# Rintazero/ft8_demodulator

Hardware: AMD Instinct MI355X
Metric: 15-s FT8 slots/sec (full decode) + LDPC candidates/sec, 1/2/4/8 MI355X (higher is better)
Workload: dtype f32 (STFT, sync score) / f64 (LLR, BP); 1 GPU; BASELINE config 3: batch of 256 independent 15-s slots per GPU, 12 kHz, K=300 candidates, min_score=2, 20 BP iterations (config 5 shape at N>1); slots_per_gpu=256, max_candidates=300, min_score=2, pipeline_depth=2, parallelism=slot-sharded x1

## Files before the change

### ft8_demodulator_amd/csrc/bp.hip

```cpp
#include "ft8_internal.h"
#include "heap_replay.h"

namespace ft8 {
namespace {

__constant__ uint16_t kChkStartD[FT8_LDPC_M + 1] = FT8_CHK_START_INIT;
__constant__ uint8_t kEdgeVarD[FT8_LDPC_E] = FT8_EDGE_VAR_INIT;
__constant__ uint16_t kVarEdgeD[FT8_LDPC_N * 3] = FT8_VAR_EDGE_INIT;
__constant__ uint8_t kEdgeChkD[FT8_LDPC_E] = FT8_EDGE_CHK_INIT;
constexpr int kGrayD[8] = {0, 1, 3, 2, 5, 6, 4, 7};

constexpr int kEdgeSlots = (FT8_LDPC_E + kWave - 1) / kWave;
constexpr int kVarSlots = (FT8_LDPC_N + kWave - 1) / kWave;
constexpr int kChkSlots = (FT8_LDPC_M + kWave - 1) / kWave;

constexpr int kDivGroup = 3;
static_assert(kEdgeSlots % kDivGroup == 0 && kVarSlots == kDivGroup, "division groups tile the slots exactly");
constexpr int kProdGroup = 3;
static_assert(kEdgeSlots % kProdGroup == 0, "product groups tile the edge slots");
constexpr int kBpWavesPerSimd = 4;
constexpr int kBpLbWaves = 3;
constexpr int kBpGridCus = 256;
constexpr double kClip2 = 2.0 * 4.97;

typedef __attribute__((address_space(3))) const double lds_f64;
typedef __attribute__((address_space(3))) const uint64_t lds_u64;

__device__ double sqrt_rn(double x) {
  double y = __builtin_sqrt(x);
  if (!(x > 0.0) || __builtin_isinf(x)) return y;
  for (int it = 0; it < 4; ++it) {
    const double lo = __longlong_as_double(__double_as_longlong(y) - 1);
    const double hi = __longlong_as_double(__double_as_longlong(y) + 1);
    if (__builtin_fma(y, lo, -x) >= 0.0) { y = lo; continue; }
    if (__builtin_fma(y, hi, -x) < 0.0) { y = hi; continue; }
    break;
  }
  return y;
}

__device__ __forceinline__ double pymax4(double a, double b, double c, double d) {
  double m = a;
  m = b > m ? b : m;
  m = c > m ? c : m;
  m = d > m ? d : m;
  return m;
}

template <int N>
__device__ __forceinline__ void div_fast(double* q, const double* x, const double* y) {
  double r[N], e[N], m[N];
#pragma unroll
  for (int i = 0; i < N; ++i) r[i] = __builtin_amdgcn_rcp(y[i]);
#pragma unroll
  for (int i = 0; i < N; ++i) e[i] = __builtin_fma(-y[i], r[i], 1.0);
#pragma unroll
  for (int i = 0; i < N; ++i) r[i] = __builtin_fma(r[i], e[i], r[i]);
#pragma unroll
  for (int i = 0; i < N; ++i) e[i] = __builtin_fma(-y[i], r[i], 1.0);
#pragma unroll
  for (int i = 0; i < N; ++i) r[i] = __builtin_fma(r[i], e[i], r[i]);
#pragma unroll
  for (int i = 0; i < N; ++i) m[i] = x[i] * r[i];
#pragma unroll
  for (int i = 0; i < N; ++i) e[i] = __builtin_fma(-y[i], m[i], x[i]);
#pragma unroll
  for (int i = 0; i < N; ++i) q[i] = __builtin_fma(e[i], r[i], m[i]);
}

template <int N, bool NEG2 = false>
__device__ __forceinline__ void div_rn(double* q, const double* x, const double* y_in, int fast = 0) {
  int ok = fast;
  if (!ok) {
    double mn = __builtin_fabs(x[0]);
#pragma unroll
    for (int i = 1; i < N; ++i) mn = __builtin_fmin(mn, __builtin_fabs(x[i]));
    ok = __ballot(mn >= 0x1p-960) == __builtin_amdgcn_read_exec() ? 1 : 0;
  }
  double r[N], e[N], m[N];
  if (ok) {
#pragma unroll
    for (int i = 0; i < N; ++i) r[i] = __builtin_amdgcn_rcp(y_in[i]);
#pragma unroll
    for (int i = 0; i < N; ++i) e[i] = __builtin_fma(-y_in[i], r[i], 1.0);
#pragma unroll
    for (int i = 0; i < N; ++i) r[i] = __builtin_fma(r[i], e[i], r[i]);
#pragma unroll
    for (int i = 0; i < N; ++i) e[i] = __builtin_fma(-y_in[i], r[i], 1.0);
#pragma unroll
    for (int i = 0; i < N; ++i) r[i] = __builtin_fma(r[i], e[i], r[i]);
#pragma unroll
    for (int i = 0; i < N; ++i) m[i] = x[i] * r[i];
#pragma unroll
    for (int i = 0; i < N; ++i) e[i] = __builtin_fma(-y_in[i], m[i], x[i]);
#pragma unroll
    for (int i = 0; i < N; ++i) q[i] = __builtin_fma(e[i], r[i], m[i]);
    return;
  }
  double den[N], num[N], y[N];
  bool f0[N], f1[N];
#pragma unroll
  for (int i = 0; i < N; ++i) y[i] = NEG2 ? -2.0 * y_in[i] : y_in[i];
#pragma unroll
  for (int i = 0; i < N; ++i) den[i] = __builtin_amdgcn_div_scale(x[i], y[i], false, &f0[i]);
#pragma unroll
  for (int i = 0; i < N; ++i) r[i] = __builtin_amdgcn_rcp(den[i]);
#pragma unroll
  for (int i = 0; i < N; ++i) num[i] = __builtin_amdgcn_div_scale(x[i], y[i], true, &f1[i]);
#pragma unroll
  for (int i = 0; i < N; ++i) e[i] = __builtin_fma(-den[i], r[i], 1.0);
#pragma unroll
  for (int i = 0; i < N; ++i) r[i] = __builtin_fma(r[i], e[i], r[i]);
#pragma unroll
  for (int i = 0; i < N; ++i) e[i] = __builtin_fma(-den[i], r[i], 1.0);
#pragma unroll
  for (int i = 0; i < N; ++i) r[i] = __builtin_fma(r[i], e[i], r[i]);
#pragma unroll
  for (int i = 0; i < N; ++i) m[i] = num[i] * r[i];
#pragma unroll
  for (int i = 0; i < N; ++i) e[i] = __builtin_fma(-den[i], m[i], num[i]);
#pragma unroll
  for (int i = 0; i < N; ++i) q[i] = __builtin_amdgcn_div_fmas(e[i], r[i], m[i], f1[i]);
#pragma unroll
  for (int i = 0; i < N; ++i) q[i] = __builtin_amdgcn_div_fixup(q[i], y[i], x[i]);
  if constexpr (NEG2) {
#pragma unroll
    for (int i = 0; i < N; ++i) q[i] = -2.0 * q[i];
  }
  (void)f0;
}

constexpr int kM7 = 24;
constexpr int kQS = FT8_LDPC_M;
constexpr int kQ6 = 6 * kQS;
constexpr int kMsgN = 584;
constexpr int kOne = kMsgN - 1;
constexpr int kHdr = 1024;
static_assert(kEdgeSlots * kWave <= kMsgN && kQ6 + kM7 == FT8_LDPC_E, "row-major message layout");

__host__ __device__ constexpr int q_of(int idx) { return idx < kQ6 ? idx / kQS : 6; }
__host__ __device__ constexpr int qa_of(int i) { return q_of(kWave * i); }
__host__ __device__ constexpr bool mixed_slot(int i) { return q_of(kWave * i + kWave - 1) != q_of(kWave * i); }
__host__ __device__ constexpr int hi_lane(int i) { return kQS * (qa_of(i) + 1) - kWave * i; }
__host__ __device__ constexpr int row_off(int i) { return 8 * (kWave * i - kQS * qa_of(i)); }

struct WaveLds {
  uint8_t bits[256];
  uint8_t a91[16];
  uint8_t rank[FT8_LDPC_M];
  uint8_t chk_of[FT8_LDPC_M];
  uint8_t pad_[kHdr - 256 - 16 - 2 * FT8_LDPC_M];
  double msg[kMsgN];
};
static_assert(offsetof(WaveLds, msg) == kHdr, "msg follows the header");

struct WaveTables {
  uint32_t va[kVarSlots], va1[kVarSlots];
  uint32_t vb[kVarSlots];
  uint32_t h[kChkSlots][kVarSlots][2];
};

__device__ __forceinline__ double ldv(uint32_t addr) {
  return *(const volatile __attribute__((address_space(3))) double*)(uintptr_t)addr;
}

__device__ __forceinline__ uint32_t lds_addr(const void* p) {
  return (uint32_t)(uintptr_t)(__attribute__((address_space(3))) const void*)p;
}

__device__ void load_tables(WaveTables& t, WaveLds& L, int lane) {
  if (lane == 0) {
    int c7 = 0, c6 = kM7;
    for (int m = 0; m < FT8_LDPC_M; ++m) {
      const int r = (kChkStartD[m + 1] - kChkStartD[m]) == 7 ? c7++ : c6++;
      L.rank[m] = (uint8_t)r;
      L.chk_of[r] = (uint8_t)m;
    }
  }
  __syncthreads();
  const uint32_t msg0 = lds_addr(&L.msg[0]);
  auto addr_of = [&](int e) -> uint32_t {
    const int m = kEdgeChkD[e], q = e - kChkStartD[m], r = L.rank[m];
    return msg0 + 8u * (uint32_t)(q < 6 ? q * kQS + r : kQ6 + r);
  };
#pragma unroll
  for (int j = 0; j < kVarSlots; ++j) {
    const int n = lane + kWave * j;
    if (n < FT8_LDPC_N) {
      t.va[j] = addr_of(kVarEdgeD[3 * n]);
      t.va1[j] = addr_of(kVarEdgeD[3 * n + 1]);
      t.vb[j] = addr_of(kVarEdgeD[3 * n + 2]);
    } else {
      const uint32_t one = msg0 + 8u * kOne;
      t.va[j] = t.va1[j] = one;
      t.vb[j] = one;
    }
  }
#pragma unroll
  for (int k = 0; k < kChkSlots; ++k) {
    const int mp = lane + kWave * k;
#pragma unroll
    for (int j = 0; j < kVarSlots; ++j) t.h[k][j][0] = t.h[k][j][1] = 0;
    if (mp < FT8_LDPC_M) {
      const int m = L.chk_of[mp];
      for (int e = kChkStartD[m]; e < kChkStartD[m + 1]; ++e) {
        const int v = kEdgeVarD[e];
#pragma unroll
        for (int j = 0; j < kVarSlots; ++j)
#pragma unroll
          for (int w = 0; w < 2; ++w)
            if (v >> 5 == 2 * j + w) t.h[k][j][w] |= 1u << (v & 31);
      }
    }
  }
  for (int x = FT8_LDPC_E + lane; x < kMsgN; x += kWave) L.msg[x] = 1.0;
  __syncthreads();
#pragma unroll
  for (int j = 0; j < kVarSlots; ++j) asm volatile("" : "+v"(t.va[j]), "+v"(t.vb[j]));
#pragma unroll
  for (int j = 0; j < kVarSlots; ++j) asm volatile("" : "+v"(t.va1[j]));
#pragma unroll
  for (int k = 0; k < kChkSlots; ++k)
#pragma unroll
    for (int j = 0; j < kVarSlots; ++j) asm volatile("" : "+v"(t.h[k][j][0]), "+v"(t.h[k][j][1]));
}

struct BpArgs {
  const void* wf;
  int wf_f64, T, F, sps, bpt, num_blocks;
  const int32_t* cand;
  const double* cand_score;
  const int32_t* cand_count;
  int N, n_items, mode, n_slots;
  const double* llr_in;
  int normalize, max_iterations;
  double* llr_out;
  uint8_t* plain_out;
  ft8_result* res;
  unsigned long long* work;
  unsigned long long work_base;
  unsigned long long* stats;
  unsigned long long* clock;
  int slot0;
  int tie_blocks;
  TieArgs tie;
};

__device__ bool tie_order(const TieArgs& a, int slot) {
  if (slot >= a.n_slots) return false;
  const int w = a.warn[slot];
  if (!(w & 8)) return false;
  const int lane = threadIdx.x, N = a.N;
  const int nsel = __builtin_amdgcn_readfirstlane(a.cand_count[slot]);
  int32_t* t = a.tie + (int64_t)slot * tie_stride(N);
  const int32_t* push = t;
  const int32_t* sel = t + N;
  int32_t* perm = t + 2 * N;
  int32_t* mi = t + 3 * N;
  int32_t* mp = t + 4 * N;
  int32_t* mk = t + 5 * N;
  const int rec = t[7 * N];
  const float* psc = reinterpret_cast<const float*>(t + 7 * N + 2);
  const double* ssc = a.cand_score + (int64_t)slot * N;
  unsigned hh[kReplayRegs], hl[kReplayRegs];
  heap_load(psc, push, nsel, hh, hl);
  int tie = heap_pushes(nsel, hh, hl);
  if (rec >= 0) tie |= heap_record(nsel, hh, hl, mono_neg(__int_as_float(t[7 * N + 1])), (unsigned)rec);

  int M = 0;
  for (int i0 = 0; i0 < nsel; i0 += kWave) {
    const int i = i0 + lane;
    unsigned key = 0, idx = 0;
    bool mem = false;
    if (i < nsel) {
      idx = (unsigned)sel[i];
      key = mono_neg((float)ssc[i]);
      mem = (i > 0 && mono_neg((float)ssc[i - 1]) == key) || (i + 1 < nsel && mono_neg((float)ssc[i + 1]) == key);
    }
    unsigned long long b = __ballot(mem);
    while (b) {
      const int l = __ffsll((long long)b) - 1;
      b &= b - 1;
      const unsigned sl = rdl(idx, l), kl = rdl(key, l);
      unsigned P = 0;
#pragma unroll
      for (int k = 0; k < kReplayRegs; ++k) {
        const int pos = 64 * k + lane;
        const unsigned long long m = __ballot(pos >= 1 && pos <= nsel && hl[k] == sl);
        if (m) P = 64u * k + (unsigned)(__ffsll((long long)m) - 1);
      }
      if (lane == 0) {
        mi[M] = i0 + l;
        mp[M] = (int)P;
        mk[M] = (int)kl;
      }
      ++M;
    }
  }
  for (int i = lane; i < nsel; i += kWave) perm[i] = i;
  __syncthreads();
  for (int m = lane; m < M; m += kWave) {
    const int i = mi[m], P = mp[m], K = mk[m];
    int below_i = 0, below_p = 0;
    for (int j = 0; j < M; ++j) {
      if (mk[j] == K) {
        below_i += mi[j] < i;
        below_p += mp[j] < P;
      }
    }
    perm[i - below_i + below_p] = i;
  }
  if (lane == 0 && tie) a.warn[slot] = w | 1;
  return true;
}

__global__ __launch_bounds__(kWave) void k_tie_apply(TieArgs a, int32_t* cand, double* cand_score) {
  const int slot = blockIdx.x, lane = threadIdx.x, N = a.N;
  if (!tie_order(a, slot)) return;
  __syncthreads();
  const int nsel = a.cand_count[slot];
  int32_t* t = a.tie + (int64_t)slot * tie_stride(N);
  const int32_t* perm = t + 2 * N;
  int32_t* stage = t + 3 * N;
  int32_t* cs = cand + (int64_t)slot * N * 2;
  double* ss = cand_score + (int64_t)slot * N;
  for (int i = lane; i < nsel; i += kWave) {
    const int src = perm[i];
    stage[4 * i] = cs[2 * src];
    stage[4 * i + 1] = cs[2 * src + 1];
    const long long v = __double_as_longlong(ss[src]);
    stage[4 * i + 2] = (int32_t)v;
    stage[4 * i + 3] = (int32_t)(v >> 32);
  }
  __syncthreads();
  for (int i = lane; i < nsel; i += kWave) {
    cs[2 * i] = stage[4 * i];
    cs[2 * i + 1] = stage[4 * i + 1];
    ss[i] = __longlong_as_double(((long long)stage[4 * i + 3] << 32) | (unsigned)stage[4 * i + 2]);
  }
}

constexpr int kLlrCpw = 4;
constexpr int kLlrRow = FT8_LDPC_N + 2;

__device__ double pairwise174x4(const double (*x)[kLlrRow], double (*part)[16], int lane) {
  const int u = lane >> 4, l = lane & 15;
  const double* xu = x[u];
  double r;
  if (l < 8) {
    r = xu[l];
    for (int i = 8; i < 80; i += 8) r += xu[i + l];
  } else {
    const int j = l - 8;
    r = xu[80 + j];
    for (int i = 8; i < 88; i += 8) r += xu[80 + i + j];
  }
  part[u][l] = r;
  __syncthreads();
  double tot = 0.0;
  if (l == 0) {
    const double* pu = part[u];
    const double s1 = ((pu[0] + pu[1]) + (pu[2] + pu[3])) + ((pu[4] + pu[5]) + (pu[6] + pu[7]));
    double s2 = ((pu[8] + pu[9]) + (pu[10] + pu[11])) + ((pu[12] + pu[13]) + (pu[14] + pu[15]));
    for (int i = 168; i < 174; ++i) s2 += xu[i];
    tot = 0.0 + (s1 + s2);
  }
  __syncthreads();
  return __shfl(tot, lane & ~15);
}

template <typename T>
__device__ void extract_llr_x4(const BpArgs& a, const int (&slot)[kLlrCpw], const int (&at)[kLlrCpw],
                               const int (&af)[kLlrCpw], int n_on, double (*c)[kLlrRow], T (*stage)[64 * 8],
                               int lane) {
  const int i = lane & 7, g = lane >> 3;
  const T* wf0 = reinterpret_cast<const T*>(a.wf);
  T v[kLlrCpw][8];
#pragma unroll
  for (int u = 0; u < kLlrCpw; ++u) {
    const int base = floordiv(at[u], a.sps);
    const T* wf = wf0 + (int64_t)slot[u] * a.T * a.F;
#pragma unroll
    for (int r = 0; r < 8; ++r) {
      const int k = 8 * r + g;
      const int sym = k + (k < 29 ? 7 : 14);
      const int block = base + sym;
      v[u][r] = (T)0;
      if (u < n_on && k < 58 && !(block < 0 || block >= a.num_blocks))
        v[u][r] = wf[(int64_t)(at[u] + sym * a.sps) * a.F + af[u] + i * a.bpt];
    }
  }
#pragma unroll
  for (int u = 0; u < kLlrCpw; ++u)
#pragma unroll
    for (int r = 0; r < 8; ++r) stage[u][8 * (8 * r + g) + i] = v[u][r];
  __syncthreads();
  if (lane < 58) {
    const int k = lane;
    const int sym = k + (k < 29 ? 7 : 14);
#pragma unroll
    for (int u = 0; u < kLlrCpw; ++u) {
      if (u >= n_on) break;
      const int block = floordiv(at[u], a.sps) + sym;
      double l0 = 0.0, l1 = 0.0, l2 = 0.0;
      if (!(block < 0 || block >= a.num_blocks)) {
        double s[8], s2[8];
#pragma unroll
        for (int j = 0; j < 8; ++j) s[j] = (double)stage[u][8 * k + j];
#pragma unroll
        for (int j = 0; j < 8; ++j) s2[j] = s[kGrayD[j]];
        l0 = pymax4(s2[4], s2[5], s2[6], s2[7]) - pymax4(s2[0], s2[1], s2[2], s2[3]);
        l1 = pymax4(s2[2], s2[3], s2[6], s2[7]) - pymax4(s2[0], s2[1], s2[4], s2[5]);
        l2 = pymax4(s2[1], s2[3], s2[5], s2[7]) - pymax4(s2[0], s2[2], s2[4], s2[6]);
      }
      c[u][3 * k] = l0;
      c[u][3 * k + 1] = l1;
      c[u][3 * k + 2] = l2;
    }
  }
}

template <typename T>
__global__ __launch_bounds__(kWave) void k_llr(BpArgs a) {
  __shared__ double c[kLlrCpw][kLlrRow];
  __shared__ double part[kLlrCpw][16];
  __shared__ double bc[kLlrCpw];
  constexpr size_t kScratch = sizeof(T) * kLlrCpw * 64 * 8 > sizeof(double) * kLlrCpw * kLlrRow
                                  ? sizeof(T) * kLlrCpw * 64 * 8 : sizeof(double) * kLlrCpw * kLlrRow;
  __shared__ __attribute__((aligned(16))) unsigned char scratch[kScratch];
  double (*sq)[kLlrRow] = reinterpret_cast<double (*)[kLlrRow]>(scratch);
  const int lane = threadIdx.x;
  if ((int)blockIdx.x < a.tie_blocks) {
    tie_order(a.tie, blockIdx.x);
    return;
  }
  const int id = blockIdx.x - a.tie_blocks;
  int item0, n_on;
  int slot[kLlrCpw] = {0, 0, 0, 0}, at[kLlrCpw] = {0, 0, 0, 0}, af[kLlrCpw] = {0, 0, 0, 0};
  static_assert(kLlrCpw == 4, "four candidates per wave");
  if (a.mode == 0) {
    const int groups = (a.N + kLlrCpw - 1) / kLlrCpw;
    const int q = id >> 3;
    const int s0 = (q / groups) * 8 + (id & 7);
    const int c0 = (q % groups) * kLlrCpw;
    if (s0 >= a.n_slots) return;
    n_on = min(kLlrCpw, min(a.N, a.cand_count[s0]) - c0);
    item0 = s0 * a.N + c0;
#pragma unroll
    for (int u = 0; u < kLlrCpw; ++u) {
      slot[u] = s0;
      if (u < n_on) {
        at[u] = a.cand[((int64_t)item0 + u) * 2];
        af[u] = a.cand[((int64_t)item0 + u) * 2 + 1];
      }
    }
  } else {
    item0 = id * kLlrCpw;
    n_on = min(kLlrCpw, a.n_items - item0);
    if (a.mode == 1) {
#pragma unroll
      for (int u = 0; u < kLlrCpw; ++u) {
        if (u < n_on) {
          slot[u] = a.cand[((int64_t)item0 + u) * 3];
          at[u] = a.cand[((int64_t)item0 + u) * 3 + 1];
          af[u] = a.cand[((int64_t)item0 + u) * 3 + 2];
        }
      }
    }
  }
  if (n_on <= 0) return;
  if (a.mode == 2) {
    for (int e = lane; e < n_on * FT8_LDPC_N; e += kWave) {
      const int u = e / FT8_LDPC_N, n = e - u * FT8_LDPC_N;
      c[u][n] = a.llr_in[(int64_t)(item0 + u) * FT8_LDPC_N + n];
    }
  } else {
    extract_llr_x4<T>(a, slot, at, af, n_on, c, reinterpret_cast<T (*)[64 * 8]>(scratch), lane);
  }
  __syncthreads();
  if (a.normalize) {
    const double mean = pairwise174x4(c, part, lane) / 174.0;
    if ((lane & 15) == 0) bc[lane >> 4] = mean;
    __syncthreads();
    for (int e = lane; e < n_on * FT8_LDPC_N; e += kWave) {
      const int u = e / FT8_LDPC_N, n = e - u * FT8_LDPC_N;
      const double d = c[u][n] - bc[u];
      sq[u][n] = d * d;
    }
    __syncthreads();
    const double var = pairwise174x4(sq, part, lane) / 174.0;
    if ((lane & 15) == 0) bc[lane >> 4] = sqrt_rn(24.0 / var);
    __syncthreads();
    for (int e = lane; e < n_on * FT8_LDPC_N; e += kWave) {
      const int u = e / FT8_LDPC_N, n = e - u * FT8_LDPC_N;
      a.llr_out[(int64_t)(item0 + u) * FT8_LDPC_N + n] = c[u][n] * bc[u];
    }
    return;
  }
  for (int e = lane; e < n_on * FT8_LDPC_N; e += kWave) {
    const int u = e / FT8_LDPC_N, n = e - u * FT8_LDPC_N;
    a.llr_out[(int64_t)(item0 + u) * FT8_LDPC_N + n] = c[u][n];
  }
}

__device__ __forceinline__ void sweep_sync() { asm volatile("" ::: "memory"); }

__device__ __forceinline__ double clip2(double T, bool nan_in) {
  const double y = __builtin_fmin(__builtin_fmax(T, -kClip2), kClip2);
  return (nan_in && T != T) ? T : y;
}

__device__ __forceinline__ void tanh_group(double* v, int fast = 0) {
  double na[kDivGroup], nb[kDivGroup];
#pragma unroll
  for (int i = 0; i < kDivGroup; ++i) {
    const double yv = v[i], z = yv * yv;
    na[i] = yv * (15120.0 + z * (420.0 + z));
    nb[i] = -30240.0 + z * (-3360.0 + z * -30.0);
  }
  int ok = fast;
  if (!ok) {
    double mn = INFINITY;
#pragma unroll
    for (int i = 0; i < kDivGroup; ++i) mn = __builtin_fmin(mn, __builtin_fabs(na[i]));
    ok = __ballot(mn >= 0x1p-480) == __builtin_amdgcn_read_exec() ? 1 : 0;
  }
  if (ok) {
    div_fast<kDivGroup>(v, na, nb);
  } else {
#pragma unroll
    for (int i = 0; i < kDivGroup; ++i) {
      const double xv = -0.5 * v[i], x2 = xv * xv;
      na[i] = xv * (945.0 + x2 * (105.0 + x2));
      nb[i] = 945.0 + x2 * (420.0 + x2 * 15.0);
    }
    div_rn<kDivGroup>(v, na, nb);
  }
}

__device__ __forceinline__ float min3_abs_hi(double a, double b, double c) {
  float m;
  asm("v_min3_f32 %0, |%1|, |%2|, |%3|"
      : "=v"(m)
      : "v"(__double2hiint(a)), "v"(__double2hiint(b)), "v"(__double2hiint(c)));
  return m;
}

__device__ __forceinline__ bool sweep_fast(const double (&y)[kVarSlots][3]) {
  static_assert(kVarSlots == 3, "three variable slots");
  const float m0 = min3_abs_hi(y[0][0], y[0][1], y[0][2]);
  const float m1 = min3_abs_hi(y[1][0], y[1][1], y[1][2]);
  const float m2 = min3_abs_hi(y[2][0], y[2][1], y[2][2]);
  float m;
  asm("v_min3_f32 %0, %1, %2, %3" : "=v"(m) : "v"(m0), "v"(m1), "v"(m2));
  const float thr = __int_as_float(923 << 20);
  return __ballot(m < thr) == 0;
}

__device__ __forceinline__ void atanh_group(double* v, int fast = 0) {
  double na[kDivGroup], nb[kDivGroup];
#pragma unroll
  for (int i = 0; i < kDivGroup; ++i) {
    const double xv = v[i], x2 = xv * xv;
    na[i] = xv * (945.0 + x2 * __builtin_fma(x2, 64.0, -735.0));
    nb[i] = (-472.5 + x2 * (525.0 + x2 * -112.5));
  }
  div_rn<kDivGroup, true>(v, na, nb, fast);
}

__device__ __forceinline__ void check_products(double* x, uint32_t la, int lane) {
#pragma unroll
  for (int i = 0; i < kEdgeSlots; ++i) {
    const int qa = qa_of(i);
    const bool mx = mixed_slot(i);
    const bool hi = mx && lane >= hi_lane(i);
    const uint32_t rb = hi ? la - 664u : la;
    double p = 0.0;
    bool first = true;
#pragma unroll
    for (int f = 0; f < 7; ++f) {
      double t;
      if (mx && f == qa) {
        const uint32_t pa = hi ? rb : rb + 664u;
        t = ldv(pa + (uint32_t)(row_off(i) + 664 * qa));
      } else if (mx && f == qa + 1) {
        continue;
      } else if (!mx && f == qa) {
        continue;
      } else {
        t = ldv(rb + (uint32_t)(row_off(i) + 664 * f));
      }
      p = first ? t : p * t;
      first = false;
    }
    x[i] = p;
    if (i % kProdGroup == kProdGroup - 1) asm volatile("" ::: "memory");
  }
}

template <bool NANSAFE>
__global__ __launch_bounds__(kWave, kBpLbWaves) void k_bp(BpArgs a) {
  const unsigned long long clk0 = a.clock ? clock64() : 0ull, wall0 = a.clock ? wall_clock64() : 0ull;
  __shared__ WaveLds L;
  const int lane = threadIdx.x;
  WaveTables tb;
  load_tables(tb, L, lane);
  const bool var2 = lane + kWave * (kVarSlots - 1) < FT8_LDPC_N;
  const uint64_t var2_mask = (1ull << (FT8_LDPC_N - kWave * (kVarSlots - 1))) - 1ull;
  uint32_t la = lds_addr(&L.msg[0]) + 8u * (uint32_t)lane;
  asm volatile("" : "+v"(la));

  unsigned st_cand = 0, st_iter = 0, st_pass = 0, st_conv = 0;
  for (;;) {
    unsigned long long ticket = 0;
    if (lane == 0) ticket = atomicAdd(a.work, 1ull);
    const unsigned lo = __builtin_amdgcn_readfirstlane((unsigned)ticket);
    const unsigned hi = __builtin_amdgcn_readfirstlane((unsigned)(ticket >> 32));
    const unsigned long long rel = (((unsigned long long)hi << 32) | lo) - a.work_base;
    if (rel >= (unsigned long long)a.n_items) break;
    const unsigned item = (unsigned)rel;

    int slot = 0, at = 0, af = 0, cidx = 0;
    double score = 0.0;
    if (a.mode == 0) {
      slot = item / a.N;
      cidx = item % a.N;
      if (cidx >= a.cand_count[slot]) continue;
      at = a.cand[((int64_t)slot * a.N + cidx) * 2];
      af = a.cand[((int64_t)slot * a.N + cidx) * 2 + 1];
      score = a.cand_score[(int64_t)slot * a.N + cidx];
    }
    double cv_[kVarSlots];
#pragma unroll
    for (int j = 0; j < kVarSlots; ++j) {
      const int n = lane + kWave * j;
      cv_[j] = n < FT8_LDPC_N ? a.llr_in[(int64_t)item * FT8_LDPC_N + n] : -1.0;
    }

    const bool nan_in = NANSAFE && __ballot(cv_[0] != cv_[0] || cv_[1] != cv_[1] || cv_[2] != cv_[2]) != 0;

#pragma unroll
    for (int i = 0; i < kEdgeSlots; ++i)
      if (i < kEdgeSlots - 1 || lane + kWave * i < FT8_LDPC_E)
        *(__attribute__((address_space(3))) double*)(uintptr_t)(la + 512u * i) = 0.0;
    __syncthreads();
    uint64_t hd[kVarSlots] = {0, 0, 0};
    int min_errors = FT8_LDPC_M;
    int entered = 0, passes = 0;
    for (int iter = 0; iter < a.max_iterations; ++iter) {
      entered++;
#pragma unroll
      for (int j = 0; j < kVarSlots; ++j) asm volatile("" : "+v"(tb.va[j]), "+v"(tb.vb[j]));
      double y[kVarSlots][3];
      const bool sweep0 = iter == 0;
      if (sweep0) {
#pragma unroll
        for (int j = 0; j < kVarSlots; ++j) {
          const double T = cv_[j] + 0.0;
          hd[j] = __ballot(T > 0.0);
          y[j][0] = y[j][1] = y[j][2] = clip2(T, nan_in);
        }
      } else {
#pragma unroll
        for (int j = 0; j < kVarSlots; ++j) {
          const double t0 = *(lds_f64*)(uintptr_t)tb.va[j];
          const double t1 = *(lds_f64*)(uintptr_t)tb.va1[j];
          const double t2 = *(lds_f64*)(uintptr_t)tb.vb[j];
          const double c = cv_[j];
          hd[j] = __ballot((c + ((t0 + t1) + t2)) > 0.0);
          const double c0 = c + t0;
          y[j][0] = (c + t1) + t2;
          y[j][1] = c0 + t2;
          y[j][2] = c0 + t1;
        }
        if (nan_in) {
#pragma unroll
          for (int j = 0; j < kVarSlots; ++j)
#pragma unroll
            for (int e = 0; e < 3; ++e) y[j][e] = clip2(y[j][e], true);
        } else {
#pragma unroll
          for (int j = 0; j < kVarSlots; ++j)
#pragma unroll
            for (int e = 0; e < 3; ++e) y[j][e] = clip2(y[j][e], false);
        }
      }
      hd[kVarSlots - 1] &= var2_mask;
      if ((hd[0] | hd[1] | hd[2]) == 0) break;
      int errs = 0;
#pragma unroll
      for (int k = 0; k < kChkSlots; ++k) {
        uint32_t x = 0;
#pragma unroll
        for (int j = 0; j < kVarSlots; ++j) {
          x = __builtin_amdgcn_bitop3_b32(tb.h[k][j][0], (uint32_t)hd[j], x, 0x6a);
          x = __builtin_amdgcn_bitop3_b32(tb.h[k][j][1], (uint32_t)(hd[j] >> 32), x, 0x6a);
        }
        errs += __popcll(__ballot(__builtin_popcount(x) & 1));
      }
      if (errs < min_errors) {
        min_errors = errs;
        if (errs == 0) break;
      }
      if (iter + 1 == a.max_iterations) break;
      static_assert(kDivGroup == 3 && kVarSlots == 3, "a division group is one variable's edges");
      int fast = __builtin_amdgcn_readfirstlane(sweep_fast(y) ? 1 : 0);
      asm volatile("" : "+s"(fast));
      if (sweep0) {
        double v[kVarSlots] = {y[0][0], y[1][0], y[2][0]};
        tanh_group(v, fast);
#pragma unroll
        for (int j = 0; j < kVarSlots; ++j) y[j][0] = y[j][1] = y[j][2] = v[j];
      }
#pragma unroll
      for (int j = 0; j < kVarSlots; ++j) {
        if (!sweep0) tanh_group(y[j], fast);
        if (j < kVarSlots - 1 || var2) {
          *(__attribute__((address_space(3))) double*)(uintptr_t)tb.va[j] = y[j][0];
          *(__attribute__((address_space(3))) double*)(uintptr_t)tb.va1[j] = y[j][1];
          *(__attribute__((address_space(3))) double*)(uintptr_t)tb.vb[j] = y[j][2];
        }
        asm volatile("" ::: "memory");
      }
      sweep_sync();
      double x[kEdgeSlots];
      check_products(x, la, lane);
#pragma unroll
      for (int g = 0; g < kEdgeSlots; g += kDivGroup) atanh_group(&x[g], fast);
#pragma unroll
      for (int i = 0; i < kEdgeSlots; ++i)
        if (i < kEdgeSlots - 1 || lane + kWave * i < FT8_LDPC_E)
          *(__attribute__((address_space(3))) double*)(uintptr_t)(la + 512u * i) = x[i];
      passes++;
      sweep_sync();
    }
    const bool pack = a.res && min_errors == 0;
    if (a.plain_out || pack) {
#pragma unroll
      for (int j = 0; j < kVarSlots; ++j) L.bits[lane + kWave * j] = (uint8_t)((hd[j] >> lane) & 1u);
      __syncthreads();
    }
    st_cand++;
    st_iter += entered;
    st_pass += passes;
    st_conv += min_errors == 0;


    if (a.plain_out)
      for (int n = lane; n < FT8_LDPC_N; n += kWave) a.plain_out[(int64_t)item * FT8_LDPC_N + n] = L.bits[n];
    if (a.res) {
      if (pack && lane < 12) {
        const uint64_t w = *reinterpret_cast<const uint64_t*>(&L.bits[8 * lane]);
        const uint32_t lo = (uint32_t)w, hi = (uint32_t)(w >> 32);
        unsigned byte = 0;
#pragma unroll
        for (int j = 0; j < 4; ++j) byte |= ((lo >> (8 * j)) & 1u) << (7 - j);
#pragma unroll
        for (int j = 0; j < 4; ++j) byte |= ((hi >> (8 * j)) & 1u) << (3 - j);
        if (lane == 11) byte &= 0xE0u;
        L.a91[lane] = (uint8_t)byte;
      }
      __syncthreads();
      if (lane == 0) {
        ft8_result r;
        r.score = score;
        r.slot = a.slot0 + slot;
        r.abs_time = at;
        r.abs_freq = af;
        r.ldpc_errors = (int16_t)min_errors;
        r.cand_index = (uint16_t)cidx;
        r.crc_extracted = 0;
        r.crc_calculated = 0;
        r.ok = 0;
        r.pass_index = 0;
        for (int i = 0; i < 10; ++i) r.payload[i] = 0;
        if (min_errors == 0) {
          const uint8_t* a91 = L.a91;
          const unsigned ce = ((a91[9] & 7u) << 11) | ((unsigned)a91[10] << 3) | (a91[11] >> 5);
          uint8_t buf[12];
          for (int i = 0; i < 10; ++i) buf[i] = a91[i];
          buf[9] &= 0xF8;
          buf[10] = 0;
          buf[11] = 0;
          unsigned rem = 0;
          for (int ib = 0; ib < 82; ++ib) {
            if ((ib & 7) == 0) rem ^= (unsigned)buf[ib >> 3] << 6;
            rem = (rem & 0x2000u) ? ((rem << 1) ^ 0x2757u) : (rem << 1);
          }
          const unsigned cc = rem & 0x3FFFu;
          r.crc_extracted = (uint16_t)ce;
          r.crc_calculated = (uint16_t)cc;
          if (ce == cc) {
            r.ok = 1;
            for (int i = 0; i < 10; ++i) r.payload[i] = a91[i];
            r.payload[9] &= 0xF8;
          }
        }
        a.res[item] = r;
      }
    }
    __syncthreads();
  }
  const unsigned row = (blockIdx.x & (unsigned)(kStatRows - 1)) * (unsigned)kStatStride;
  if (a.stats && lane == 0 && st_cand) {
    atomicAdd(&a.stats[row + 0], (unsigned long long)st_cand);
    atomicAdd(&a.stats[row + 1], (unsigned long long)st_iter);
    atomicAdd(&a.stats[row + 2], (unsigned long long)st_pass);
    atomicAdd(&a.stats[row + 3], (unsigned long long)st_conv);
  }
  if (a.clock && lane == 0) {
    const unsigned long long cyc = clock64() - clk0, wall = wall_clock64() - wall0;
    atomicAdd(&a.clock[row + 0], cyc);
    atomicAdd(&a.clock[row + 1], wall);
    atomicMax(&a.clock[row + 2], cyc);
    atomicAdd(&a.clock[row + 3], 1ull);
  }
}

__global__ __launch_bounds__(kWave) void k_compact(const ft8_result* res, const int32_t* cand_count,
                                                   int N, ft8_result* out, int32_t* counts, int cap,
                                                   const int32_t* warn, const int32_t* tie) {
  const int slot = blockIdx.x, lane = threadIdx.x;
  const int nc = cand_count[slot];
  const int32_t* perm = (tie && (warn[slot] & 8)) ? tie + (int64_t)slot * tie_stride(N) + 2 * N : nullptr;
  const ft8_result* rs = res + (int64_t)slot * N;
  int base = 0;
  for (int c0 = 0; c0 < nc; c0 += kWave) {
    const int c = c0 + lane;
    const int src = c < nc ? (perm ? perm[c] : c) : 0;
    const bool ok = c < nc && rs[src].ok;
    const unsigned long long m = __ballot(ok);
    const int pos = base + __popcll(m & ((1ull << lane) - 1ull));
    if (ok && pos < cap) {
      out[(int64_t)slot * cap + pos] = rs[src];
      if (perm) out[(int64_t)slot * cap + pos].cand_index = (uint16_t)c;
    }
    base += __popcll(m);
  }
  if (lane == 0) counts[slot] = base;
}

constexpr int kPackThreads = 1024;
__global__ __launch_bounds__(kPackThreads) void k_pack(const ft8_result* rec, const int32_t* counts, int n_slots,
                                                       int cap, int capacity, int slot_offset, uint8_t* send,
                                                       ft8_result* overflow) {
  FT8_RACE_PROLOGUE();
  __shared__ int s_off[kPackThreads];
  __shared__ int s_wave[kPackThreads / kWave + 1];
  const int tid = threadIdx.x, lane = tid & (kWave - 1), w = tid >> 6;
  int32_t* cnt_out = reinterpret_cast<int32_t*>(send + 8);
  ft8_result* rows = reinterpret_cast<ft8_result*>(send + pack_header_bytes(n_slots));
  int carry = 0;
  for (int base = 0; base < n_slots; base += kPackThreads) {
    const int s = base + tid;
    int c = 0;
    if (s < n_slots) {
      const int raw = counts[s];
      cnt_out[s] = raw;
      c = min(max(raw, 0), cap);
    }
    int x = c;
#pragma unroll
    for (int o = 1; o < kWave; o <<= 1) {
      const int y = __shfl_up(x, o);
      if (lane >= o) x += y;
    }
    if (lane == kWave - 1) s_wave[w] = x;
    __syncthreads();
    if (tid == 0) {
      int acc = 0;
      for (int i = 0; i < kPackThreads / kWave; ++i) {
        const int t = s_wave[i];
        s_wave[i] = acc;
        acc += t;
      }
      s_wave[kPackThreads / kWave] = acc;
    }
    __syncthreads();
    s_off[tid] = s < n_slots ? s_wave[w] + x - c : 0x7fffffff;
    const int ct = s_wave[kPackThreads / kWave];
    __syncthreads();
    for (int r = tid; r < ct; r += kPackThreads) {
      int lo = 0, hi = min(kPackThreads, n_slots - base) - 1;
      while (lo < hi) {
        const int mid = (lo + hi + 1) >> 1;
        if (s_off[mid] <= r) lo = mid;
        else hi = mid - 1;
      }
      ft8_result v = rec[(int64_t)(base + lo) * cap + (r - s_off[lo])];
      v.slot += slot_offset;
      const int dst = carry + r;
      if (dst < capacity) rows[dst] = v;
      else if (overflow) overflow[dst - capacity] = v;
    }
    carry += ct;
    __syncthreads();
  }
  for (int r = carry + tid; r < capacity; r += kPackThreads) {
    uint64_t* p = reinterpret_cast<uint64_t*>(rows + r);
#pragma unroll
    for (int i = 0; i < (int)(sizeof(ft8_result) / 8); ++i) p[i] = 0;
  }
  for (int i = n_slots + tid; i < (int)((pack_header_bytes(n_slots) - 8) / 4); i += kPackThreads) cnt_out[i] = 0;
  if (tid == 0) *reinterpret_cast<int64_t*>(send) = carry;
}

__global__ void k_crc14(const uint8_t* msg, const int32_t* nbits, int n, uint16_t* crc) {
  const int i = blockIdx.x * blockDim.x + threadIdx.x;
  if (i >= n) return;
  const uint8_t* m = msg + (int64_t)i * 12;
  const int nb = nbits[i];
  unsigned rem = 0;
  for (int b = 0; b < nb; ++b) {
    if ((b & 7) == 0) rem ^= (unsigned)m[b >> 3] << 6;
    rem = (rem & 0x2000u) ? ((rem << 1) ^ 0x2757u) : (rem << 1);
  }
  crc[i] = (uint16_t)(rem & 0x3FFFu);
}

__global__ void k_ldpc_check(const uint8_t* bits, int n, int32_t* err) {
  const int i = blockIdx.x * blockDim.x + threadIdx.x;
  if (i >= n) return;
  const uint8_t* b = bits + (int64_t)i * FT8_LDPC_N;
  int e = 0;
  for (int m = 0; m < FT8_LDPC_M; ++m) {
    int x = 0;
    for (int j = kChkStartD[m]; j < kChkStartD[m + 1]; ++j) x ^= b[kEdgeVarD[j]];
    e += x != 0;
  }
  err[i] = e;
}

BpArgs make_args(const BpLaunch& L) {
  BpArgs a{};
  a.wf = L.wf;
  a.wf_f64 = L.wf_f64;
  a.T = L.T;
  a.F = L.F;
  a.sps = L.sps;
  a.bpt = L.bpt;
  a.num_blocks = L.sps > 0 ? L.T / L.sps : 0;
  a.cand = L.cand;
  a.cand_score = L.cand_score;
  a.cand_count = L.cand_count;
  a.N = L.N;
  a.n_items = L.n_items;
  a.n_slots = L.n_slots;
  a.mode = L.mode;
  a.llr_in = L.llr_in;
  a.normalize = L.normalize;
  a.max_iterations = L.max_iterations;
  a.llr_out = L.llr_out;
  a.plain_out = L.plain_out;
  a.res = L.res;
  a.work = L.work;
  a.work_base = L.work_base ? *L.work_base : 0ull;
  a.stats = L.stats;
  a.clock = L.clock;
  a.slot0 = L.slot0;
  a.tie = TieArgs{L.n_slots, L.N, L.cand_count, L.warn, L.tie, L.cand_score};
  a.tie_blocks = (L.tie && L.mode == 0) ? (L.n_slots + 7) / 8 * 8 : 0;
  return a;
}

}

hipError_t launch_llr(const BpLaunch& L, hipStream_t s) {
  if (L.n_items <= 0) return hipSuccess;
  BpArgs a = make_args(L);
  const int64_t grid = a.tie_blocks + (L.mode == 0 ? (int64_t)((L.n_slots + 7) / 8) * 8 * ((L.N + kLlrCpw - 1) / kLlrCpw)
                                                    : ((int64_t)L.n_items + kLlrCpw - 1) / kLlrCpw);
  if (L.wf_f64)
    hipLaunchKernelGGL(k_llr<double>, dim3((unsigned)grid), dim3(kWave), 0, s, a);
  else
    hipLaunchKernelGGL(k_llr<float>, dim3((unsigned)grid), dim3(kWave), 0, s, a);
  return hipGetLastError();
}

hipError_t launch_bp(const BpLaunch& L, hipStream_t s) {
  if (L.n_items <= 0) return hipSuccess;
  BpArgs a = make_args(L);
  const int per_simd = max(1, min(L.grid_waves, kBpWavesPerSimd));
  const int waves = min(L.n_items, kBpGridCus * 4 * per_simd);
  if (L.mode == 0) hipLaunchKernelGGL(k_bp<false>, dim3(waves), dim3(kWave), 0, s, a);
  else hipLaunchKernelGGL(k_bp<true>, dim3(waves), dim3(kWave), 0, s, a);
  const hipError_t e = hipGetLastError();
  if (e == hipSuccess && L.work_base) *L.work_base += (unsigned long long)L.n_items + (unsigned long long)waves;
  return e;
}

hipError_t launch_tie_apply(const TieArgs& a, int32_t* cand, double* cand_score, hipStream_t s) {
  if (a.n_slots <= 0 || !a.tie) return hipSuccess;
  hipLaunchKernelGGL(k_tie_apply, dim3(a.n_slots), dim3(kWave), 0, s, a, cand, cand_score);
  return hipGetLastError();
}

hipError_t launch_compact(const CompactLaunch& L, hipStream_t s) {
  if (L.n_slots <= 0) return hipSuccess;
  hipLaunchKernelGGL(k_compact, dim3(L.n_slots), dim3(kWave), 0, s, L.res, L.cand_count, L.N, L.out,
                     L.counts, L.cap, L.warn, L.tie);
  return hipGetLastError();
}

hipError_t launch_pack(const ft8_result* rec, const int32_t* counts, int n_slots, int cap, int capacity,
                       int slot_offset, uint8_t* send, ft8_result* overflow, hipStream_t s) {
  static_assert(sizeof(ft8_result) % 8 == 0, "records are copied as 8-byte words");
  hipLaunchKernelGGL(k_pack, dim3(1), dim3(kPackThreads), 0, s, rec, counts, n_slots, cap, capacity, slot_offset,
                     send, overflow);
  return hipGetLastError();
}

hipError_t launch_crc14(const uint8_t* msg, const int32_t* nbits, int n, uint16_t* crc, hipStream_t s) {
  if (n <= 0) return hipSuccess;
  hipLaunchKernelGGL(k_crc14, dim3((n + 255) / 256), dim3(256), 0, s, msg, nbits, n, crc);
  return hipGetLastError();
}

hipError_t launch_ldpc_check(const uint8_t* bits, int n, int32_t* err, hipStream_t s) {
  if (n <= 0) return hipSuccess;
  hipLaunchKernelGGL(k_ldpc_check, dim3((n + 255) / 256), dim3(256), 0, s, bits, n, err);
  return hipGetLastError();
}

}
```

Before: 136,500 slots/s.

## Compute LDPC check-node products check-major with prefix/suffix sharing per row

Replaces the edge-major check-product loop, where each lane formed every extrinsic product from six separate LDS loads, with a check-major mapping. Each lane owns one of the first 64 check rows, loads its seven messages once and builds all leave-one-out products with shared prefix/suffix products. The 19 leftover degree-6 rows are split across 57 lanes, with a constexpr validator proving every edge is written exactly once. This cuts LDS reads and multiplies per sweep, at the cost of extra live registers and uneven lane work on the leftover rows.

```diff
diff --git a/ft8_demodulator_amd/csrc/bp.hip b/ft8_demodulator_amd/csrc/bp.hip
--- a/ft8_demodulator_amd/csrc/bp.hip
+++ b/ft8_demodulator_amd/csrc/bp.hip
@@ -16,8 +16,6 @@
 
 constexpr int kDivGroup = 3;
 static_assert(kEdgeSlots % kDivGroup == 0 && kVarSlots == kDivGroup, "division groups tile the slots exactly");
-constexpr int kProdGroup = 3;
-static_assert(kEdgeSlots % kProdGroup == 0, "product groups tile the edge slots");
 constexpr int kBpWavesPerSimd = 4;
 constexpr int kBpLbWaves = 3;
 constexpr int kBpGridCus = 256;
@@ -138,11 +136,43 @@
 constexpr int kHdr = 1024;
 static_assert(kEdgeSlots * kWave <= kMsgN && kQ6 + kM7 == FT8_LDPC_E, "row-major message layout");
 
-__host__ __device__ constexpr int q_of(int idx) { return idx < kQ6 ? idx / kQS : 6; }
-__host__ __device__ constexpr int qa_of(int i) { return q_of(kWave * i); }
-__host__ __device__ constexpr bool mixed_slot(int i) { return q_of(kWave * i + kWave - 1) != q_of(kWave * i); }
-__host__ __device__ constexpr int hi_lane(int i) { return kQS * (qa_of(i) + 1) - kWave * i; }
-__host__ __device__ constexpr int row_off(int i) { return 8 * (kWave * i - kQS * qa_of(i)); }
+constexpr int kLeftRows = FT8_LDPC_M - kWave;
+constexpr int kLeftLanes = 3 * kLeftRows;
+constexpr int kRowB = 8 * kQS;
+static_assert(kWave + kLeftRows == FT8_LDPC_M && kLeftRows == 19, "64 + 19 rows");
+static_assert(kM7 <= kWave, "every leftover row has degree 6");
+static_assert(kLeftLanes <= kWave, "3 x 19 leftover lanes fit the wave");
+static_assert(kQ6 + kWave - 1 < kMsgN, "a check-major lane's seventh factor is a message or a constant");
+static_assert(kEdgeSlots == 7 + 2, "seven check-major products and two leftover ones per lane");
+__host__ __device__ constexpr int left_q3(int lane) { return lane / kLeftRows < 3 ? lane / kLeftRows : 2; }
+__host__ __device__ constexpr int left_r(int lane) { return lane % kLeftRows; }
+__host__ __device__ constexpr int left_f0(int q3) { return q3 == 0 ? 1 : 0; }
+__host__ __device__ constexpr int left_f1(int q3) { return q3 == 2 ? 1 : 2; }
+__host__ __device__ constexpr int msg_idx(int q, int mp) { return q * kQS + mp; }
+__host__ __device__ constexpr bool phase_d_mapping_ok() {
+  int stores[kMsgN] = {};
+  for (int lane = 0; lane < kWave; ++lane) {
+    for (int f = 0; f < 7; ++f) {
+      if (msg_idx(f, lane) >= kMsgN) return false;
+      if (f < 6 || lane < kM7) stores[msg_idx(f, lane)]++;
+    }
+    const int q3 = left_q3(lane), row = kWave + left_r(lane);
+    for (int s = 0; s < 2; ++s) {
+      const int fs[5] = {3 * s + left_f0(q3), 3 * s + left_f1(q3), 3 * (1 - s), 3 * (1 - s) + 1, 3 * (1 - s) + 2};
+      int seen = 0;
+      for (int k = 0; k < 5; ++k) {
+        if (fs[k] < 0 || fs[k] > 5 || row >= FT8_LDPC_M || msg_idx(fs[k], row) >= kQ6) return false;
+        seen |= 1 << fs[k];
+      }
+      if (seen != (0x3f & ~(1 << (3 * s + q3)))) return false;
+      if (lane < kLeftLanes) stores[msg_idx(3 * s + q3, row)]++;
+    }
+  }
+  for (int x = 0; x < kMsgN; ++x)
+    if (stores[x] != (x < FT8_LDPC_E ? 1 : 0)) return false;
+  return true;
+}
+static_assert(phase_d_mapping_ok(), "phase D reads inside msg and produces every edge exactly once");
 
 struct WaveLds {
   uint8_t bits[256];
@@ -568,34 +598,50 @@
   div_rn<kDivGroup, true>(v, na, nb, fast);
 }
 
-__device__ __forceinline__ void check_products(double* x, uint32_t la, int lane) {
-#pragma unroll
-  for (int i = 0; i < kEdgeSlots; ++i) {
-    const int qa = qa_of(i);
-    const bool mx = mixed_slot(i);
-    const bool hi = mx && lane >= hi_lane(i);
-    const uint32_t rb = hi ? la - 664u : la;
-    double p = 0.0;
-    bool first = true;
-#pragma unroll
-    for (int f = 0; f < 7; ++f) {
-      double t;
-      if (mx && f == qa) {
-        const uint32_t pa = hi ? rb : rb + 664u;
-        t = ldv(pa + (uint32_t)(row_off(i) + 664 * qa));
-      } else if (mx && f == qa + 1) {
-        continue;
-      } else if (!mx && f == qa) {
-        continue;
-      } else {
-        t = ldv(rb + (uint32_t)(row_off(i) + 664 * f));
-      }
-      p = first ? t : p * t;
-      first = false;
-    }
-    x[i] = p;
-    if (i % kProdGroup == kProdGroup - 1) asm volatile("" ::: "memory");
-  }
+struct LeftAddr {
+  uint32_t rb, f0, f1, st;
+};
+
+__device__ __forceinline__ LeftAddr left_addr(uint32_t msg0, int lane) {
+  const int q3 = left_q3(lane);
+  LeftAddr a;
+  a.rb = msg0 + 8u * (uint32_t)(kWave + left_r(lane));
+  a.f0 = a.rb + (uint32_t)(kRowB * left_f0(q3));
+  a.f1 = a.rb + (uint32_t)(kRowB * left_f1(q3));
+  a.st = a.rb + (uint32_t)(kRowB * q3);
+  return a;
+}
+
+__device__ __forceinline__ void row_products(double* x, uint32_t la) {
+  double t[7];
+#pragma unroll
+  for (int f = 0; f < 7; ++f) t[f] = ldv(la + (uint32_t)(kRowB * f));
+  double p = t[1];
+#pragma unroll
+  for (int f = 2; f < 7; ++f) p *= t[f];
+  x[0] = p;
+  double pre = t[0];
+#pragma unroll
+  for (int q = 1; q < 7; ++q) {
+    p = pre;
+#pragma unroll
+    for (int f = q + 1; f < 7; ++f) p *= t[f];
+    x[q] = p;
+    pre *= t[q];
+  }
+}
+
+__device__ __forceinline__ void left_products(double* x, const LeftAddr& a) {
+  double p = ldv(a.f0) * ldv(a.f1);
+#pragma unroll
+  for (int f = 3; f < 6; ++f) p *= ldv(a.rb + (uint32_t)(kRowB * f));
+  x[0] = p;
+  p = ldv(a.rb);
+#pragma unroll
+  for (int f = 1; f < 3; ++f) p *= ldv(a.rb + (uint32_t)(kRowB * f));
+  p *= ldv(a.f0 + (uint32_t)(kRowB * 3));
+  p *= ldv(a.f1 + (uint32_t)(kRowB * 3));
+  x[1] = p;
 }
 
 template <bool NANSAFE>
@@ -609,6 +655,8 @@
   const uint64_t var2_mask = (1ull << (FT8_LDPC_N - kWave * (kVarSlots - 1))) - 1ull;
   uint32_t la = lds_addr(&L.msg[0]) + 8u * (uint32_t)lane;
   asm volatile("" : "+v"(la));
+  LeftAddr lf = left_addr(la - 8u * (uint32_t)lane, lane);
+  asm volatile("" : "+v"(lf.rb), "+v"(lf.f0), "+v"(lf.f1), "+v"(lf.st));
 
   unsigned st_cand = 0, st_iter = 0, st_pass = 0, st_conv = 0;
   for (;;) {
@@ -724,13 +772,19 @@
       }
       sweep_sync();
       double x[kEdgeSlots];
-      check_products(x, la, lane);
+      row_products(x, la);
+      left_products(&x[7], lf);
 #pragma unroll
       for (int g = 0; g < kEdgeSlots; g += kDivGroup) atanh_group(&x[g], fast);
 #pragma unroll
-      for (int i = 0; i < kEdgeSlots; ++i)
-        if (i < kEdgeSlots - 1 || lane + kWave * i < FT8_LDPC_E)
-          *(__attribute__((address_space(3))) double*)(uintptr_t)(la + 512u * i) = x[i];
+      for (int f = 0; f < 6; ++f)
+        *(__attribute__((address_space(3))) double*)(uintptr_t)(la + (uint32_t)(kRowB * f)) = x[f];
+      if (lane < kM7)
+        *(__attribute__((address_space(3))) double*)(uintptr_t)(la + (uint32_t)(kRowB * 6)) = x[6];
+      if (lane < kLeftLanes) {
+        *(__attribute__((address_space(3))) double*)(uintptr_t)lf.st = x[7];
+        *(__attribute__((address_space(3))) double*)(uintptr_t)(lf.st + (uint32_t)(kRowB * 3)) = x[8];
+      }
       passes++;
       sweep_sync();
     }
```

Result: faster. 146,000 slots/s (median of 6 runs) (+7.0%).
